# endernewton/tf-faster-rcnn

Measured on AMD Instinct MI355X. Metric: images/sec (600×1000) ResNet-101 Faster R-CNN at 1/2/4/8 MI355X, higher is better.
Workload: dtype f32 (operands, accumulators, results; GEMMs with Cin, Cout % 128 == 0 form each f32 product from two-piece fp16 operands with an exact power-of-two scale per 128-k block on the fp16 matrix pipe -- 3 MFMAs / product, dropped terms <= 3 * 2^-22, measured error vs float64 below the f32-MFMA kernel's; o

## Files before the change

### include/frcnn_hip.h

```cpp
#ifndef FRCNN_HIP_H_
#define FRCNN_HIP_H_
#include <stddef.h>
#include <stdint.h>

#ifdef __cplusplus
extern "C" {
#endif

#define FRCNN_OK 0
#define FRCNN_E_ARG (-1)
#define FRCNN_E_WS (-2)
#define FRCNN_E_UNSUPPORTED (-3)
#define FRCNN_E_HIP(e) (-(1000 + (int)(e)))

#define FRCNN_NMS_RULE_CPU 0
#define FRCNN_NMS_RULE_GPU 1

#define FRCNN_ACT_NONE 0
#define FRCNN_ACT_RELU 1
#define FRCNN_ACT_RELU6 2

#define FRCNN_ABI_VERSION 6
int frcnn_abi_version(void);
const char* frcnn_build_info(void);
// ... 87 lines not shown
size_t frcnn_conv2d_workspace_bytes(int N, int OH, int OW, int Cout, int KH, int KW, int Cin, int fold_w);
int frcnn_conv2d_nhwc_ws(const float* x_d, int N, int H, int W, int Cin, const float* w_d, const float* bias_d,
                         const float* residual_d, int RH, int RW, int res_stride, float* y_d, int OH, int OW, int Cout, int KH,
                         int KW, int stride, int pad_top, int pad_left, int act, int fold_w, void* ws, size_t ws_bytes,
                         void* stream);

int frcnn_set_tuning(int key, int value);
unsigned int frcnn_crc32c(const void* data, size_t n, unsigned int crc);

long long frcnn_snappy_uncompress(const unsigned char* src, size_t n, unsigned char* dst, size_t cap);

int frcnn_prep_image_shape(int h, int w, int target_size, int max_size, double* im_scale, int* out_h, int* out_w);
int frcnn_prep_image(const void* src_d, int src_is_float, int h, int w, const double* pixel_means, double im_scale, float* out_d,
                     int OH, int OW, int out_c, void* stream);
int frcnn_prep_train_image(const void* src_d, int src_is_float, int h, int w, int flipped, const double* pixel_means, double im_scale,
                           float* out_d, int OH, int OW, int out_c, const unsigned short* boxes_d, const int* classes_d, int G,
                           float* gt_d, void* stream);

int frcnn_gemm_batched_nt(const float* x_d, const float* w_d, float* y_d, int G, int M, int N, int K, void* stream);
size_t frcnn_gemm_x3_pack_bytes(int G, int N, int K);
int frcnn_gemm_x3_pack(const float* w_d, int G, int N, int K, void* planes_d, void* stream);
int frcnn_gemm_x3(const float* x_d, const void* planes_d, const float* bias_d, const float* res_d, float* y_d, int G, int M, int N,
                  int K, int act, int cfg, int terms, void* stream);
size_t frcnn_h2_planes_bytes(long long rows, int K);
int frcnn_h2_pack_w(const float* w_d, int G, int N, int K, void* planes_d, float* w_inv_d, void* stream);
int frcnn_h2_split(const float* x_d, long long M, int K, void* planes_d, float* inv_d, void* stream);
int frcnn_gemm_h2(const void* x_planes_d, const float* x_inv_d, const void* w_planes_d, const float* w_inv_d, const float* bias_d,
                  const float* res_d, const void* res_planes_d, const float* res_inv_d, float* y_d, void* y_planes_d, float* y_inv_d,
                  int G, int M, int N, int K, int act, int cfg, void* stream);
size_t frcnn_gemm_h2_mean_workspace_bytes(int G, int M, int N);
int frcnn_gemm_h2_mean(const void* x_planes_d, const float* x_inv_d, const void* w_planes_d, const float* w_inv_d, const float* bias_d,
                       const float* res_d, const void* res_planes_d, const float* res_inv_d, int G, int M, int N, int K, int act, int rows,
                       float* mean_out_d, void* ws, size_t ws_bytes, int cfg, void* stream);
int frcnn_winograd_filter_transform(const float* w_hwio, int Cin, int Cout, const float* scale, int m, float* u_out);
int frcnn_winograd_filter_transform_device(const float* w_packed_d, int Cout, int Cin, int m, int transpose_flip, float* u_d,
                                           void* stream);
int frcnn_winograd_input_transform(const float* x_d, int N, int H, int W, int C, int m, float* v_d, void* stream);
int frcnn_winograd_output_transform(const float* m_d, int N, int H, int W, int C, int m, const float* bias_d, int act, float* y_d,
                                    void* stream);
int frcnn_winograd7_filter_transform(const float* w_hwio, int Cin, int Cout, const float* scale, float* u_out);
int frcnn_winograd7_filter_transform_device(const float* w_packed_d, int Cout, int Cin, int transpose_flip, float* u_d, void* stream);
int frcnn_winograd7_input_transform(const float* x_d, int R, int C, float* v_d, void* stream);
int frcnn_winograd7_output_transform(const float* m_d, int R, int C, const float* bias_d, int act, float* y_d, void* stream);
int frcnn_winograd_input_transform_h2(const float* x_d, int N, int H, int W, int C, int m, void* v_planes_d, float* v_inv_d, void* stream);
int frcnn_winograd_output_transform_h2(const float* m_d, int N, int H, int W, int C, int m, const float* bias_d, int act, float* y_d,
                                       void* y_planes_d, float* y_inv_d, void* stream);
// ... 114 lines not shown
```

### tf-faster-rcnn_amd/csrc/gemm_h2.hip

```cpp
#include "h2_common.h"
#include <mutex>
#include <type_traits>

typedef float f32x16 __attribute__((ext_vector_type(16)));
typedef _Float16 h8 __attribute__((ext_vector_type(8)));

#define LDS_AS __attribute__((address_space(3)))

struct GemmH2Params {
  const unsigned short* x; const float* x_inv; const unsigned short* w; const float* w_inv;
  const float* bias; const float* res; const unsigned short* resp; const float* resp_inv; float* y; unsigned short* yp; float* y_inv;
  int M, N, K, batch, act, nsteps, mtiles, ntiles;
  long long Mtot;
  int wshare;
  const float* mask;
  float* mean_part; int mean_rows;
};

__device__ __forceinline__ void h2_glds16(unsigned voff, const void* sbase, unsigned lds_base) {
  unsigned keep;
  asm volatile(
      "s_mov_b32 %0, m0\n\t"
      "s_mov_b32 m0, %3\n\t"
      "s_nop 0\n\t"
// ... 1088 lines not shown
                                    const float* res_d, const float* mask_d, float* y_d, void* y_planes_d, float* y_inv_d, int G, int M, int N, int K,
                                    int act, int cfg, void* stream) {
  if (!x_planes_d || !x_inv_d || !w_planes_d || !w_inv_d || !mask_d || (!y_d && !y_planes_d) || (y_planes_d && !y_inv_d) || G <= 0 || M <= 0 ||
      N <= 0 || K <= 0 || act < 0 || act > 2)
    return FRCNN_E_ARG;
  const long long Mtot = (long long)G * M;
  if (K % H2_KB || N % 128 || 4ll * Mtot * K >= (1ll << 32) || 4ll * N * K >= (1ll << 32) || (long long)M * N >= (1ll << 29)) return FRCNN_E_UNSUPPORTED;
  GemmH2Params p = h2_params(x_planes_d, x_inv_d, w_planes_d, w_inv_d, bias_d, res_d, nullptr, nullptr, y_d, y_planes_d, y_inv_d, G, M, N, K, act);
  p.mask = mask_d;
  return run_h2(p, cfg, (hipStream_t)stream);
}

static int run_h2(GemmH2Params& p, int cfg, hipStream_t st) {
  const int G = p.batch, M = p.M, N = p.N, K = p.K;
  if (cfg < 0) {
    const long long mt256 = (M + 255) / 256;
#ifndef FRCNN_H2_PP_MIN_K
#define FRCNN_H2_PP_MIN_K 1024
#endif
    const int pp_min_k = ((cfg == -4 || cfg == -5 || cfg == -6) && !p.mean_part) ? 512 : FRCNN_H2_PP_MIN_K;
    const int pp_cfg = (cfg == -3 || cfg == -4 || (cfg == -6 && K < FRCNN_H2_PP_MIN_K)) ? 34 : 21;
    const bool pp = K >= pp_min_k && mt256 * 256 * 100 <= (long long)M * 104 && mt256 * (N / 128) * G >= 256;
    const bool tiny = (long long)((M + 127) / 128) * (N / 128) * G < 150;
    const bool de = cfg != -2 && cfg != -7 && !p.mean_part && !p.mask && ((p.resp && p.yp && !p.y) || cfg == -8);
    cfg = pp ? pp_cfg : tiny ? (cfg == -2 ? 12 : (de && cfg == -8) ? 41 : 33) : (cfg == -2 ? 9 : de ? 40 : 31);
  }
  if (p.mean_part && (cfg == 40 || cfg == 41)) cfg = cfg == 40 ? 31 : 33;
  return p.mask ? h2_dispatch<H2_MASKED>(p, cfg, st) : h2_dispatch<0>(p, cfg, st);
}

__global__ __launch_bounds__(256) void k_h2_mean_finish(const float* __restrict__ part, int G, int M, int N4, int rows, float4* __restrict__ out) {
  const long long t = (long long)blockIdx.x * blockDim.x + threadIdx.x;
  const int per = M / rows;
  if (t >= (long long)G * per * N4) return;
  const int n4 = (int)(t % N4);
  const long long gr = t / N4;
  const int g = (int)(gr / per), r = (int)(gr % per);
  const int nblk = (M + 31) >> 5;
  const int row0 = r * rows, row1 = row0 + rows - 1;
  float4 s = make_float4(0.f, 0.f, 0.f, 0.f);
  for (int b = row0 >> 5; b <= (row1 >> 5); ++b) {
    const int which = ((b << 5) / rows == r) ? 0 : 1;
    const float4 v = *(const float4*)(part + (((size_t)g * nblk + b) * 2 + which) * (size_t)N4 * 4 + (size_t)n4 * 4);
    s.x += v.x; s.y += v.y; s.z += v.z; s.w += v.w;
  }
  const float inv = 1.0f / (float)rows;
  out[t] = make_float4(s.x * inv, s.y * inv, s.z * inv, s.w * inv);
// ... 28 lines not shown
```

### tf-faster-rcnn_amd/csrc/gemm_x3.hip

```cpp
#include "common.h"
#include "mfma_f32.h"
#include <mutex>

typedef __attribute__((ext_vector_type(8))) __bf16 bf16x8;

struct GemmX3Params {
  const float* x; const unsigned short* wp; const float* bias; const float* res; float* y;
  int M, N, K, nsteps, mtiles, ntiles, batch, act;
  long long gx, gwp, gy;
};

__device__ __forceinline__ void x3_split8(const float4 a, const float4 b, bf16x8& h, bf16x8& m, bf16x8& l) {
  const float v[8] = {a.x, a.y, a.z, a.w, b.x, b.y, b.z, b.w};
#pragma unroll
  for (int q = 0; q < 8; ++q) {
    const __bf16 hq = (__bf16)v[q];
    const float r = v[q] - (float)hq;
    const __bf16 mq = (__bf16)r;
    const float s = r - (float)mq;
    h[q] = hq; m[q] = mq; l[q] = (__bf16)s;
  }
}

template <int BM, int BN, int WM, int WN, int TERMS = 6>
__global__ __launch_bounds__((BM / WM) * (BN / WN) * 64) __attribute__((amdgpu_waves_per_eu(2))) void k_gemm_x3(const GemmX3Params p) {
  constexpr int NW = (BM / WM) * (BN / WN);
  constexpr int TM = WM / 32, TN = WN / 32;
  constexpr int LA = BM / 8 / NW;
  constexpr int LB = 3 * BN / 16 / NW;
  constexpr int G = LA + LB;
  constexpr int A_BYTES = BM * 128, P_BYTES = BN * 64, STAGE = A_BYTES + 3 * P_BYTES;
  static_assert((BM / 8) % NW == 0 && (3 * BN / 16) % NW == 0, "tile/wave mismatch");
  extern __shared__ __attribute__((aligned(16))) char smem[];

  const int tid = threadIdx.x, lane = tid & 63;
  const int wave = __builtin_amdgcn_readfirstlane(tid >> 6);
  const int per = p.mtiles * p.ntiles, T = per * p.batch;
  const int xcd = blockIdx.x & 7, wx = blockIdx.x >> 3, W8 = gridDim.x >> 3;
  const int tq = T / 8, tr = T % 8, tn = tq + (xcd < tr ? 1 : 0);
  const int t_end = (xcd < tr ? xcd * (tq + 1) : tr * (tq + 1) + (xcd - tr) * tq) + tn;
  int tile = __builtin_amdgcn_readfirstlane(t_end - tn + wx);
  if (tile >= t_end) return;

  const int wm0 = (wave / (BN / WN)) * WM, wn0 = (wave % (BN / WN)) * WN;
  int a_lane[LA], b_lane[LB];
#pragma unroll
  for (int t = 0; t < LB; ++t) {
    const int u = wave * LB + t;
    const int plane = u / (BN / 16), row = (u % (BN / 16)) * 16 + (lane >> 2), pos = lane & 3;
    b_lane[t] = ((plane * p.N + row) * p.K) * 2 + ((pos ^ ((row >> 2) & 3)) * 16);
  }
  const float* ia = p.x; const char* ib = (const char*)p.wp;
  int i_bm0 = 0, i_bn0 = 0, i_g = 0;
  auto set_tile = [&](int tl) {
    const int g = tl / per, rem = tl - g * per;
    const int mt = rem / p.ntiles, nt = rem - mt * p.ntiles;
    i_bm0 = mt * BM; i_bn0 = nt * BN; i_g = g;
    ia = p.x + (size_t)g * p.gx + (size_t)i_bm0 * p.K;
    ib = (const char*)(p.wp + (size_t)g * p.gwp + (size_t)i_bn0 * p.K);
#pragma unroll
    for (int t = 0; t < LA; ++t) {
      const int row = (wave * LA + t) * 8 + (lane >> 3);
      a_lane[t] = (min(row, p.M - 1 - i_bm0) * p.K + ((lane & 7) ^ ((row >> 1) & 7)) * 4) * 4;
    }
  };
  const unsigned lds0 = (unsigned)(size_t)(LDS_AS char*)smem;
  auto issue_one = [&](int buf, int t) {
    const unsigned sb = lds0 + (unsigned)(buf * STAGE);
    if (t < LA) glds16((const char*)ia + a_lane[t], __builtin_amdgcn_readfirstlane(sb + (wave * LA + t) * 1024));
    else glds16(ib + b_lane[t - LA], __builtin_amdgcn_readfirstlane(sb + A_BYTES + (wave * LB + (t - LA)) * 1024));
  };
  auto advance_k = [&]() { ia += 32; ib += 64; };
  auto issue_slab = [&](int buf) {
#pragma unroll
    for (int t = 0; t < G; ++t) issue_one(buf, t);
    advance_k();
  };

  f32x16 acc[TM][TN], acs[TM][TN];
  auto zero_acc = [&]() {
#pragma unroll
    for (int i = 0; i < TM; ++i)
#pragma unroll
      for (int j = 0; j < TN; ++j)
#pragma unroll
        for (int r = 0; r < 16; ++r) { acc[i][j][r] = 0.f; acs[i][j][r] = 0.f; }
  };
  zero_acc();
  const int frow = lane & 31, khalf = lane >> 5;
  const int a_sw = (frow >> 1) & 7, b_sw = (frow >> 2) & 3;
  const int a_row = (wm0 + frow) * 128, b_row = A_BYTES + (wn0 + frow) * 64;

  int c_bm0, c_bn0, c_g;
  const int lane_off = (4 * khalf * p.N + frow) * 4;
  auto sub_base = [&](int i, int j) { return (long long)(c_bm0 + wm0 + i * 32) * p.N + (long long)(c_bn0 + wn0 + j * 32); };
// ... 32 lines not shown
          acs[i][j] = __builtin_amdgcn_mfma_f32_32x32x16_bf16(al[i], bh[j], acs[i][j], 0, 0, 0);
          acc[i][j] = __builtin_amdgcn_mfma_f32_32x32x16_bf16(ah[i], bh[j], acc[i][j], 0, 0, 0);
          acs[i][j] = __builtin_amdgcn_mfma_f32_32x32x16_bf16(ah[i], bl[j], acs[i][j], 0, 0, 0);
          acs[i][j] = __builtin_amdgcn_mfma_f32_32x32x16_bf16(am[i], bm[j], acs[i][j], 0, 0, 0);
          acs[i][j] = __builtin_amdgcn_mfma_f32_32x32x16_bf16(am[i], bh[j], acs[i][j], 0, 0, 0);
          acs[i][j] = __builtin_amdgcn_mfma_f32_32x32x16_bf16(ah[i], bm[j], acs[i][j], 0, 0, 0);
          if (TERMS == 9) {
            acs[i][j] = __builtin_amdgcn_mfma_f32_32x32x16_bf16(al[i], bl[j], acs[i][j], 0, 0, 0);
            acs[i][j] = __builtin_amdgcn_mfma_f32_32x32x16_bf16(al[i], bm[j], acs[i][j], 0, 0, 0);
            acs[i][j] = __builtin_amdgcn_mfma_f32_32x32x16_bf16(am[i], bl[j], acs[i][j], 0, 0, 0);
          }
        }
    }
    advance_k();
  };

  const float act_lo = p.act == FRCNN_ACT_NONE ? -__builtin_inff() : 0.f;
  const float act_hi = p.act == FRCNN_ACT_RELU6 ? 6.f : __builtin_inff();
  auto finish = [&](auto res_c) {
    constexpr bool RES = decltype(res_c)::value;
    float* const py = p.y + (size_t)c_g * p.gy;
    int lo = lane_off;
    asm volatile("" : "+v"(lo));
#pragma unroll
    for (int i = 0; i < TM; ++i)
#pragma unroll
      for (int j = 0; j < TN; ++j) {
        const float bv = p.bias ? p.bias[c_bn0 + wn0 + j * 32 + frow] : 0.f;
        const long long sbase = sub_base(i, j);
        float v[16];
        if (RES) {
          const auto rr = rsrc_of(p.res + (size_t)c_g * p.gy, sbase);
#pragma unroll
          for (int r = 0; r < 16; ++r) v[r] = __builtin_bit_cast(float, __builtin_amdgcn_raw_buffer_load_b32(rr, lo + row_soff(r), 0, 0));
        }
#pragma unroll
        for (int r = 0; r < 16; ++r) {
          float t = (acc[i][j][r] + acs[i][j][r]) + bv;
          if (RES) t += v[r];
          v[r] = act_clamp(t, act_lo, act_hi);
        }
        const auto ry = rsrc_of(py, sbase);
#pragma unroll
        for (int r = 0; r < 16; ++r) __builtin_amdgcn_raw_buffer_store_b32(__builtin_bit_cast(unsigned, v[r]), ry, lo + row_soff(r), 0, 0);
      }
  };

  set_tile(tile);
  c_bm0 = i_bm0; c_bn0 = i_bn0; c_g = i_g;
  issue_slab(0);
  int cur = 0, step = 0;
  for (;;) {
    wait_vmcnt<0>();
    __builtin_amdgcn_s_barrier();
// ... 20 lines not shown
  const long long g = i / nk, e = i - g * nk;
  const float x = w[i];
  const __bf16 h = (__bf16)x;
  const float r = x - (float)h;
  const __bf16 m = (__bf16)r;
  const __bf16 l = (__bf16)(r - (float)m);
  unsigned short* o = out + (size_t)g * 3 * nk + e;
  o[0] = __builtin_bit_cast(unsigned short, h); o[nk] = __builtin_bit_cast(unsigned short, m); o[2 * nk] = __builtin_bit_cast(unsigned short, l);
}

extern "C" size_t frcnn_gemm_x3_pack_bytes(int G, int N, int K) {
  if (G <= 0 || N <= 0 || K <= 0) return 0;
  return (size_t)G * 3 * (size_t)N * (size_t)K * sizeof(unsigned short);
}

extern "C" int frcnn_gemm_x3_pack(const float* w_d, int G, int N, int K, void* planes_d, void* stream) {
  if (!w_d || !planes_d || G <= 0 || N <= 0 || K <= 0) return FRCNN_E_ARG;
  const long long nk = (long long)N * K, tot = nk * G;
  hipLaunchKernelGGL(k_x3_pack, dim3((unsigned)((tot + 255) / 256)), dim3(256), 0, (hipStream_t)stream, w_d, nk, G, (unsigned short*)planes_d);
  LAUNCH_CHECK();
  return FRCNN_OK;
}

template <int BM, int BN, int WM, int WN, int TERMS = 6>
static int launch_x3(const GemmX3Params& q, hipStream_t st) {
  constexpr int NT = (BM / WM) * (BN / WN) * 64;
  constexpr size_t lds = 2 * (size_t)(BM * 128 + 3 * BN * 64);
  auto kern = k_gemm_x3<BM, BN, WM, WN, TERMS>;
  static KernelOnce once;
  int slots = 0;
  HIP_TRY(kernel_once(once, (const void*)kern, NT, lds, &slots));
  if (slots < 8 || q.N % BN) return FRCNN_E_UNSUPPORTED;
  GemmX3Params p = q;
  p.mtiles = cdiv(p.M, BM); p.ntiles = p.N / BN; p.nsteps = p.K / 32;
  const long long T = (long long)p.mtiles * p.ntiles * p.batch;
  if (T >= (1ll << 30)) return FRCNN_E_UNSUPPORTED;
  const int grid = (int)min((long long)(slots / 8) * 8, ((T + 7) / 8) * 8);
  hipLaunchKernelGGL(kern, dim3(grid), dim3(NT), lds, st, p);
  LAUNCH_CHECK();
  return FRCNN_OK;
}

extern "C" int frcnn_gemm_x3(const float* x_d, const void* planes_d, const float* bias_d, const float* res_d, float* y_d, int G, int M,
                             int N, int K, int act, int cfg, int terms, void* stream) {
  if (!x_d || !planes_d || !y_d || G <= 0 || M <= 0 || N <= 0 || K <= 0 || act < 0 || act > 2 || (terms != 6 && terms != 9)) return FRCNN_E_ARG;
  if (K % 32 || N % 64 || (long long)M * N >= (1ll << 31) || (long long)N * K >= (1ll << 28) || K >= (1 << 22))
    return FRCNN_E_UNSUPPORTED;
  GemmX3Params p;
  p.x = x_d; p.wp = (const unsigned short*)planes_d; p.bias = bias_d; p.res = res_d; p.y = y_d;
  p.M = M; p.N = N; p.K = K; p.batch = G; p.act = act;
  p.gx = (long long)M * K; p.gwp = 3ll * N * K; p.gy = (long long)M * N;
  p.nsteps = p.mtiles = p.ntiles = 0;
  hipStream_t st = (hipStream_t)stream;
  if (cfg >= 0 && cfg < 10 && (N % 128) && cfg != 6) cfg = -1;
  if (cfg < 0)
    cfg = (N % 128) ? 6 : ((long long)cdiv(M, 128) * (N / 128) * G >= 256) ? 0 : 1;
  if (terms == 9) {
    switch (cfg) {
      case 0: return launch_x3<128, 128, 64, 64, 9>(p, st);
      case 1: return launch_x3<128, 128, 32, 64, 9>(p, st);
      case 6: return launch_x3<128, 64, 64, 32, 9>(p, st);
      default: return FRCNN_E_ARG;
    }
  }
  switch (cfg) {
    case 0: return launch_x3<128, 128, 64, 64>(p, st);
    case 1: return launch_x3<128, 128, 32, 64>(p, st);
    case 2: return launch_x3<64, 128, 32, 64>(p, st);
    case 3: return launch_x3<128, 128, 32, 128>(p, st);
    case 4: return launch_x3<256, 128, 64, 64>(p, st);
    case 5: return launch_x3<128, 256, 64, 64>(p, st);
    case 6: return launch_x3<128, 64, 64, 32>(p, st);
    default: return FRCNN_E_ARG;
  }
}
```

### tf-faster-rcnn_amd/frcnn_hip/__init__.py

```python
import ctypes
import os
from ctypes import c_double, c_float, c_int, c_longlong, c_size_t, c_ulonglong, c_void_p

_PKG = os.path.dirname(os.path.abspath(__file__))
LIB_PATH = os.path.join(_PKG, "libfrcnn_hip.so")
_lib = None

ABI_VERSION = 6
ACT_NONE, ACT_RELU, ACT_RELU6 = 0, 1, 2
NMS_RULE_CPU, NMS_RULE_GPU = 0, 1

_P = c_void_p
SIGNATURES = {
    "frcnn_abi_version": (c_int, []),
    "frcnn_build_info": (ctypes.c_char_p, []),
    "_nms": (None, [_P, _P, _P, c_int, c_int, c_float, c_int]),
    "frcnn_nms_workspace_bytes": (c_size_t, [c_int]),
    "frcnn_nms": (c_int, [_P, c_int, c_double, c_int, _P, _P, _P, c_size_t, _P]),
    "frcnn_nms_sorted": (c_int, [_P, c_int, c_int, c_double, c_int, _P, _P, _P, c_size_t, _P]),
    "frcnn_nms_rule": (c_int, [_P, c_int, c_double, c_int, c_int, _P, _P, _P, c_size_t, _P]),
    "frcnn_nms_sorted_rule": (c_int, [_P, c_int, c_int, c_double, c_int, c_int, _P, _P, _P, c_size_t, _P]),
    "frcnn_generate_anchors": (c_int, [c_int, _P, c_int, _P, c_int, _P]),
    "frcnn_generate_anchors_pre": (c_int, [c_int, c_int, c_int, _P, c_int, _P, _P]),
    "frcnn_proposal_workspace_bytes": (c_size_t, [c_int, c_int, c_int, c_int]),
# ... 75 lines not shown
    "frcnn_proposal_target_layer_dn": (c_int, [_P, _P, c_int, _P, _P, c_int, c_int, c_int, c_double, c_double, c_double, c_double, _P, _P,
                                               c_longlong, _P, _P, _P, _P, _P, _P, _P, _P, _P]),
    "frcnn_loss_workspace_bytes": (c_size_t, [c_longlong]),
    "frcnn_softmax_ce_loss": (c_int, [_P, _P, c_int, c_int, c_int, c_int, c_int, _P, _P, _P, c_size_t, _P]),
    "frcnn_smooth_l1_loss": (c_int, [_P, _P, _P, _P, c_longlong, c_float, c_float, _P, _P, _P, c_size_t, _P]),
    "frcnn_transpose_pad": (c_int, [_P, c_int, c_int, _P, c_int, _P]),
    "frcnn_im2col_t": (c_int, [_P, c_int, c_int, c_int, c_int, c_int, c_int, c_int, c_int, c_int, c_int, c_int, _P, c_int, _P]),
    "frcnn_flip_transpose_filter": (c_int, [_P, c_int, c_int, c_int, c_int, _P, _P]),
    "frcnn_conv2d_dgrad_strided": (c_int, [_P, c_int, c_int, c_int, c_int, _P, c_int, c_int, c_int, c_int, c_int, c_int, _P, c_int,
                                           c_int, c_int, _P]),
    "frcnn_conv2d_wgrad_supported": (c_int, [c_int, c_int]),
    "frcnn_conv2d_wgrad_workspace_bytes": (c_size_t, [c_int, c_int, c_int, c_int, c_int, c_int, c_int]),
    "frcnn_conv2d_wgrad": (c_int, [_P, _P, c_int, c_int, c_int, c_int, c_int, c_int, c_int, c_int, c_int, c_int, c_int, c_int, _P, _P,
                                   c_size_t, _P]),
    "frcnn_conv2d_wgrad_set_plan": (None, [c_int, c_int]),
    "frcnn_conv2d_wgrad_h2_workspace_bytes": (c_size_t, [c_int, c_int, c_int, c_int, c_int, c_int, c_int]),
    "frcnn_conv2d_wgrad_h2": (c_int, [_P, _P, c_int, c_int, c_int, c_int, c_int, c_int, c_int, c_int, c_int, c_int, c_int, c_int, _P, _P,
                                      c_size_t, _P]),
    "frcnn_conv2d_wgrad_h2_set_plan": (None, [c_int, c_int]),
    "frcnn_relu_bwd": (c_int, [_P, _P, c_longlong, _P]),
    "frcnn_gemm_x3_pack_bytes": (c_size_t, [c_int, c_int, c_int]),
    "frcnn_gemm_x3_pack": (c_int, [_P, c_int, c_int, c_int, _P, _P]),
    "frcnn_gemm_x3": (c_int, [_P, _P, _P, _P, _P, c_int, c_int, c_int, c_int, c_int, c_int, c_int, _P]),
    "frcnn_h2_planes_bytes": (c_size_t, [c_longlong, c_int]),
    "frcnn_h2_pack_w": (c_int, [_P, c_int, c_int, c_int, _P, _P, _P]),
    "frcnn_h2_split": (c_int, [_P, c_longlong, c_int, _P, _P, _P]),
    "frcnn_gemm_h2": (c_int, [_P, _P, _P, _P, _P, _P, _P, _P, _P, _P, _P, c_int, c_int, c_int, c_int, c_int, c_int, _P]),
    "frcnn_gemm_h2_mean_workspace_bytes": (c_size_t, [c_int, c_int, c_int]),
    "frcnn_gemm_h2_mean": (c_int, [_P, _P, _P, _P, _P, _P, _P, _P, c_int, c_int, c_int, c_int, c_int, c_int, _P, _P, c_size_t, c_int, _P]),
    "frcnn_relu6_bwd": (c_int, [_P, _P, c_longlong, _P]),
    "frcnn_maxpool_bwd": (c_int, [_P, c_int, c_int, c_int, c_int, c_int, c_int, _P, _P, c_int, c_int, _P, _P]),
    "frcnn_dropout": (c_int, [_P, c_longlong, c_ulonglong, c_float, _P, _P]),
    "frcnn_dwconv3x3_dgrad": (c_int, [_P, c_int, c_int, c_int, c_int, _P, _P, c_int, c_int, c_int, c_int, c_int, c_int, _P]),
    "frcnn_dwconv3x3_wgrad_workspace_bytes": (c_size_t, [c_int, c_int, c_int, c_int]),
    "frcnn_dwconv3x3_wgrad": (c_int, [_P, _P, c_int, c_int, c_int, c_int, c_int, c_int, c_int, c_int, c_int, _P, _P, _P, c_size_t, _P]),
    "frcnn_dwconv3x3_refold": (c_int, [_P, _P, c_int, _P, _P]),
    "frcnn_add_strided": (c_int, [_P, c_int, c_int, c_int, c_int, _P, c_int, c_int, c_int, c_int, _P]),
    "frcnn_spatial_mean_bwd": (c_int, [_P, c_int, c_int, c_int, _P, _P]),
    "frcnn_colsum": (c_int, [_P, c_int, c_int, _P, _P]),
    "frcnn_crop_and_resize_bwd": (c_int, [_P, c_int, c_int, c_int, _P, c_int, c_float, c_int, _P, _P]),
    "frcnn_crop_and_resize_bwd_plan": (c_int, [_P, c_int, c_int, c_int, _P, c_int, c_float, c_int, _P, c_size_t, _P]),
    "frcnn_sgd_momentum": (c_int, [_P, _P, _P, _P, _P, c_longlong, c_int, c_float, c_float, c_float, c_float, _P]),
    "frcnn_sgd_desc_bytes": (c_size_t, []),
    "frcnn_sgd_momentum_multi": (c_int, [_P, c_int, c_float, c_float, c_float, _P]),
    "frcnn_sgd_momentum_range": (c_int, [_P, c_int, c_int, c_float, c_float, c_float, _P]),
    "frcnn_sumsq": (c_int, [_P, c_longlong, c_double, _P, c_int, _P, c_size_t, _P]),
# ... 47 lines not shown
```

### tf-faster-rcnn_amd/frcnn_hip/ops.py

```python
import ctypes

import numpy as np
import torch

import frcnn_hip as _binding
from . import ACT_NONE, NMS_RULE_CPU, call, lib

_ws_cache = {}
ws_scope = "default"

_scope_stack = [(None, None, None)]


def active_store(owner, default=None):
    o, _, store = _scope_stack[-1]
    return store if store is not None and (owner is None or o is owner) else default


def scope_depth():
    return len(_scope_stack) - 1


class unscoped(object):

# ... 795 lines not shown
def relu_bwd(grad, y):
    _chk(grad), _chk(y)
    call("frcnn_relu_bwd", _ptr(grad), _ptr(y), grad.numel(), _stream())
    return grad


def gemm_x3_pack(w, planes=None):
    _chk(w)
    G, N, K = (w.shape[0], w.shape[1], w.shape[2]) if w.dim() == 3 else (1, w.shape[0], w[0].numel())
    if planes is None:
        planes = torch.empty(lib().frcnn_gemm_x3_pack_bytes(G, N, K), dtype=torch.uint8, device=w.device)
    call("frcnn_gemm_x3_pack", _ptr(w), G, N, K, _ptr(planes), _stream())
    return planes


def gemm_x3(x, planes, G, M, N, K, bias=None, residual=None, act=ACT_NONE, out=None, cfg=-1, terms=6):
    _chk(x)
    out = _empty((G, M, N) if G > 1 else (M, N), dtype=torch.float32, device=x.device) if out is None else out
    call("frcnn_gemm_x3", _ptr(x), _ptr(planes), _ptr(bias), _ptr(residual), _ptr(out), int(G), int(M), int(N), int(K), int(act),
         int(cfg), int(terms), _stream())
    return out


class H2(object):
    __slots__ = ("planes", "inv", "rows", "K")

    def __init__(self, planes, inv, rows, K):
        self.planes, self.inv, self.rows, self.K = planes, inv, int(rows), int(K)

    @staticmethod
    def empty(rows, K, device):
        assert K % 128 == 0
        return H2(torch.empty(lib().frcnn_h2_planes_bytes(int(rows), int(K)), dtype=torch.uint8, device=device),
                  torch.empty((K // 128, rows), dtype=torch.float32, device=device), rows, K)

    def to_float(self):
        hl = self.planes.view(torch.float16).view(2, self.rows, self.K).float()
        inv = self.inv.t().repeat_interleave(128, dim=1)
        return (hl[0] + hl[1]) * inv


def h2_split(x, out=None):
    _chk(x)
    K = x.shape[-1]
    rows = x.numel() // K
    out = H2.empty(rows, K, x.device) if out is None else out
# ... 218 lines not shown
```

### tf-faster-rcnn_amd/lib/model/config.py

```python
import ast
import os
import os.path as osp

import numpy as np


class AttrDict(dict):

    def __init__(self, d=None, **kw):
        super().__init__()
        for k, v in dict(d or {}, **kw).items():
            self[k] = v

    def __setitem__(self, k, v):
        if isinstance(v, dict) and not isinstance(v, AttrDict):
            v = AttrDict(v)
        super().__setitem__(k, v)

    def __getattr__(self, k):
        try:
            return self[k]
        except KeyError:
            raise AttributeError(k)

# ... 9 lines not shown
    BBOX_INSIDE_WEIGHTS=(1.0, 1.0, 1.0, 1.0), BBOX_NORMALIZE_TARGETS_PRECOMPUTED=True,
    BBOX_NORMALIZE_MEANS=(0.0, 0.0, 0.0, 0.0), BBOX_NORMALIZE_STDS=(0.1, 0.1, 0.2, 0.2), PROPOSAL_METHOD='gt',
    HAS_RPN=True, RPN_POSITIVE_OVERLAP=0.7, RPN_NEGATIVE_OVERLAP=0.3, RPN_CLOBBER_POSITIVES=False,
    RPN_FG_FRACTION=0.5, RPN_BATCHSIZE=256, RPN_NMS_THRESH=0.7, RPN_PRE_NMS_TOP_N=12000,
    RPN_POST_NMS_TOP_N=2000, RPN_BBOX_INSIDE_WEIGHTS=(1.0, 1.0, 1.0, 1.0), RPN_POSITIVE_WEIGHT=-1.0,
    USE_ALL_GT=True)

_TEST = dict(
    SCALES=(600,), MAX_SIZE=1000, NMS=0.3, SVM=False, BBOX_REG=True, HAS_RPN=False, PROPOSAL_METHOD='gt',
    RPN_NMS_THRESH=0.7, RPN_PRE_NMS_TOP_N=6000, RPN_POST_NMS_TOP_N=300, MODE='nms', RPN_TOP_N=5000)

__C = AttrDict(
    TRAIN=_TRAIN, TEST=_TEST,
    RESNET=dict(MAX_POOL=False, FIXED_BLOCKS=1),
    MOBILENET=dict(REGU_DEPTH=False, FIXED_LAYERS=5, WEIGHT_DECAY=0.00004, DEPTH_MULTIPLIER=1.),
    PIXEL_MEANS=np.array([[[102.9801, 115.9465, 122.7717]]]), RNG_SEED=3,
    ROOT_DIR=osp.abspath(osp.join(osp.dirname(__file__), '..', '..')),
    MATLAB='matlab', EXP_DIR='default', USE_GPU_NMS=True, USE_E2E_TF=False, POOLING_MODE='crop', POOLING_SIZE=7,
    ANCHOR_SCALES=[8, 16, 32], ANCHOR_RATIOS=[0.5, 1, 2], RPN_CHANNELS=512,
    HIP=dict(WINOGRAD=True, WINOGRAD_MIN_CIN=64, WINOGRAD_M=4, WINOGRAD_F2_SCOPES=("block1", "block2"), WINOGRAD_DIRECT_SCOPES=(),
             WINOGRAD_TRAIN=True, WINOGRAD_DGRAD=True,
             WINOGRAD_7X7=True, FUSE_TAIL_MEAN=True, MFMA_X3=True,
             MFMA_H2=True, H2_LAZY_SPLIT=True, H2_MIN_TILES=150, H2_TRAIN_MIN_TILES=320, H2_TRUNK_PLANES=True, H2_TILE_CFG=-1,
             X3_TILE_CFG=-1, H2_TRAIN=True, WGRAD_STREAM=2, WGRAD_TN=True, WGRAD_H2=True, PREP_STREAM=True, TRAIN_REPLAY=True, TRAIN_PICK_STREAMS=6,
             GRAPH_CACHE_SHAPES=4, TRAIN_CACHE_SHAPES=16))
__C.DATA_DIR = osp.abspath(osp.join(__C.ROOT_DIR, 'data'))
cfg = __C


def get_output_dir(imdb, weights_filename):
    outdir = osp.abspath(osp.join(__C.ROOT_DIR, 'output', __C.EXP_DIR, imdb.name))
    outdir = osp.join(outdir, 'default' if weights_filename is None else weights_filename)
    os.makedirs(outdir, exist_ok=True)
    return outdir


def get_output_tb_dir(imdb, weights_filename):
    outdir = osp.abspath(osp.join(__C.ROOT_DIR, 'tensorboard', __C.EXP_DIR, imdb.name))
    outdir = osp.join(outdir, 'default' if weights_filename is None else weights_filename)
    os.makedirs(outdir, exist_ok=True)
    return outdir


_NULLABLE_KEYS = ("H2_TRAIN_MIN_TILES",)


def _merge_a_into_b(a, b):
# ... 56 lines not shown
```

### tf-faster-rcnn_amd/lib/nets/network.py

```python
import collections

import numpy as np
import torch

from frcnn_hip import ACT_NONE, ACT_RELU, NMS_RULE_CPU, NMS_RULE_GPU, ops
from frcnn_hip.runtime import VarSpec
from model.config import cfg


class Network(object):
    def __init__(self):
        self._predictions = {}
        self._losses = {}
        self._anchor_targets = {}
        self._proposal_targets = {}
        self._layers = {}
        self._act_summaries = []
        self._variables_to_fix = {}
        self._feat_stride = [16, ]
        self._scope = "network"
        self._sess = None
        self._image = None
        self._im_info = None
        self._var_specs = collections.OrderedDict()
# ... 71 lines not shown
                      lambda: ops.conv3x3_winograd(x, u, b, act, out=out, v_buf=v, m_buf=mm, out_planes=yp),
                      nbytes=4 * (v.numel() + u.numel() + mm.numel()))
            self._wrote(out, yp, True) if yp is not None else self._wrote(out)
        elif plain and self._h2_eligible(M, Cout, Cin, 1, scope) and self._h2_input(x) is not None:
            xp, wp = self._h2_input(x), sess.h2_planes(w)
            yp = sess.h2_buf(self._tag + "/" + scope, M, Cout) if emit_h2 else None
            y = out if (want_f32 or yp is None or self._mode == "TRAIN") else None
            res = residual
            if residual is not None and residual.data_ptr() in self._f32_missing:
                res = self._h2_of[residual.data_ptr()]
            tcfg = int(cfg.HIP.H2_TILE_CFG)
            sess.mark("conv:h2:" + scope, flops, lambda: ops.gemm_h2(xp, wp, 1, M, Cout, Cin, b, res, act, out=y, out_planes=yp,
                                                                      want_f32=False, cfg=tcfg),
                      nbytes=4 * M * Cin + 4 * w.numel() + (4 * out.numel() if y is not None else 0)
                      + (4 * out.numel() if yp is not None else 0) + (4 * out.numel() if residual is not None else 0))
            self._wrote(out, yp, y is not None)
        elif plain and self._x3_eligible(M, Cout, Cin, 1):
            self._need_f32(x), self._need_f32(residual)
            planes = sess.x3_planes(w)
            xc = int(cfg.HIP.X3_TILE_CFG)
            sess.mark("conv:x3:" + scope, flops, lambda: ops.gemm_x3(x, planes, 1, M, Cout, Cin, b, residual, act, out=out, cfg=xc),
                      nbytes=4 * (x.numel() + out.numel() + (out.numel() if residual is not None else 0)) + 6 * w.numel())
            self._wrote(out)
        else:
            self._need_f32(x), self._need_f32(residual)
            sess.mark("conv:" + scope, flops,
                      lambda: ops.conv2d(x, w, b, k, k, stride, pad, act, residual, res_stride, fold_w, out=out),
                      nbytes=4 * (x.numel() + w.numel() + out.numel() + (out.numel() if residual is not None else 0)))
            self._wrote(out)
        if self._mode == "TRAIN":
            self._tape.append(dict(kind="conv", scope=scope, x=x, y=out, k=k, stride=stride, pad=tuple(pad), act=act,
                                   residual=residual, res_stride=res_stride))
            if self.trainable_scope(scope) or x.data_ptr() in self._requires_grad:
                self._requires_grad.add(out.data_ptr())
            if residual is not None and residual.data_ptr() in self._requires_grad:
                self._requires_grad.add(out.data_ptr())
        return out

    H2_MIN_CHANNEL_RATIO = 2.0 ** -18

    def _h2_eligible(self, M, N, K, G, scope=None):
        rows = G * M
        if scope is not None and self._mode == "TEST" and self._sess.h2_channel_spread(scope) < self.H2_MIN_CHANNEL_RATIO:
            return False
        return (bool(cfg.HIP.MFMA_H2) and (self._mode == "TEST" or bool(cfg.HIP.H2_TRAIN)) and K % 128 == 0 and N % 128 == 0
                and ((self._plan_rows(M) + 127) // 128) * (N // 128) * G >= self._h2_min_tiles()
# ... 14 lines not shown
            self._need_f32(x)
            K = x.shape[-1]
            xp = self._sess.h2_buf(self._tag + "/split@%x" % x.data_ptr(), x.numel() // K, K)
            self._sess.mark("op:h2_split", 0, lambda: ops.h2_split(x, out=xp), nbytes=8 * x.numel())
            self._h2_of[x.data_ptr()] = xp
        return xp

    def _wrote(self, t, planes=None, f32=True):
        k = t.data_ptr()
        if planes is None:
            self._h2_of.pop(k, None)
        else:
            self._h2_of[k] = planes
        (self._f32_missing.discard if f32 else self._f32_missing.add)(k)
        return t

    def _need_f32(self, x):
        if x is not None and x.data_ptr() in self._f32_missing:
            raise RuntimeError("graph construction error: a float32 consumer reads a tensor that was emitted as operand planes only")

    def _x3_eligible(self, M, N, K, G):
        return (bool(cfg.HIP.MFMA_X3) and self._mode == "TEST" and N % 64 == 0 and K % 32 == 0
                and ((self._plan_rows(M) + 127) // 128) * ((N + 127) // 128) * G >= 150 and M * N < (1 << 31) and N * K < (1 << 28))

    @staticmethod
    def _winograd_scheme(scope, H, W):
        if any(tok in scope for tok in cfg.HIP.WINOGRAD_F2_SCOPES):
            return 2
        m = int(cfg.HIP.WINOGRAD_M)
        return 7 if (m == 4 and H == 7 and W == 7 and cfg.HIP.WINOGRAD_7X7) else m

    def _conv_winograd(self, x, scope, act, bn_eps, emit_h2=False, want_f32=True):
        sess = self._sess
        self._need_f32(x)
        N, H, W, Cin = x.shape
        m = self._winograd_scheme(scope, H, W)
        u, b = sess.winograd_params(scope, bn_eps=bn_eps, m=m)
        G, Cout = u.shape[0], u.shape[1]
        T = ops.winograd_tiles(N, H, W, m)
        mm = sess.buf(self._tag + "/wino_m", (G, T, Cout))
        out = sess.buf(self._tag + "/" + scope, (N, H, W, Cout))
        flops = 2 * G * T * Cout * Cin
        if self._h2_eligible(T, Cout, Cin, G, scope):
            vp, wp = sess.h2_buf(self._tag + "/wino_v", G * T, Cin), sess.h2_planes(u)
            sess.mark("op:wino_in", 0, lambda: ops.winograd_input_transform_h2(x, vp, m), nbytes=4 * (x.numel() + G * T * Cin))
            tcfg = int(cfg.HIP.H2_TILE_CFG)
# ... 353 lines not shown
        self._var(self._scope + "/bbox_pred/biases", (4 * num_classes,), "zeros")
        names = ["rois", "rpn_cls_score", "rpn_cls_prob", "rpn_bbox_pred", "cls_score", "cls_prob", "bbox_pred"]
        return {k: k for k in names}

    def _stage_image(self, sess, image, im_info=None):
        if isinstance(image, np.ndarray):
            image = torch.from_numpy(np.ascontiguousarray(image, dtype=np.float32))
        B, H, W, C = image.shape
        if im_info is None:
            buf = sess.buf(self._tag + "/image", (B, H, W, 4), zero=True)
        else:
            with self.shape_scope(sess, (B, H, W, 4), im_info):
                buf = sess.buf(self._tag + "/image", (B, H, W, 4), zero=True)
        buf[..., :C].copy_(image, non_blocking=True)
        return buf

    def graph_key(self, image_shape, im_info):
        c = cfg[self._mode]
        return (self._tag, self._scope, self._num_classes, self._anchor_scales, self._anchor_ratios, bool(cfg.RESNET.MAX_POOL),
                bool(cfg.USE_GPU_NMS), tuple(int(v) for v in image_shape), (float(im_info[0]), float(im_info[1])), self._mode, cfg.TEST.MODE, self._fuse_tail_entry,
                c.RPN_PRE_NMS_TOP_N, c.RPN_POST_NMS_TOP_N, c.RPN_NMS_THRESH, cfg.TEST.RPN_TOP_N, cfg.POOLING_SIZE,
                bool(cfg.HIP.WINOGRAD), int(cfg.HIP.WINOGRAD_MIN_CIN), int(cfg.HIP.WINOGRAD_M), tuple(cfg.HIP.WINOGRAD_F2_SCOPES),
                tuple(cfg.HIP.WINOGRAD_DIRECT_SCOPES), bool(cfg.HIP.WINOGRAD_7X7), bool(cfg.HIP.FUSE_TAIL_MEAN), bool(cfg.HIP.MFMA_X3), bool(cfg.USE_E2E_TF),
                bool(cfg.HIP.MFMA_H2), bool(cfg.HIP.H2_LAZY_SPLIT), int(cfg.HIP.H2_MIN_TILES), bool(cfg.HIP.H2_TRUNK_PLANES), int(cfg.HIP.H2_TILE_CFG), int(cfg.HIP.X3_TILE_CFG), bool(cfg.HIP.H2_TRAIN))

    def shape_scope(self, sess, image_shape, im_info):
        return sess.shape_scope(self.graph_key(image_shape, im_info), group=("graphs", self._tag), cap=int(cfg.HIP.GRAPH_CACHE_SHAPES))

    def forward_device(self, sess, image_d, im_info, use_graph=True):
        self._sess = sess
        self._image = image_d
        self._im_info = (float(im_info[0]), float(im_info[1]), float(im_info[2]))
        sess.prepared.wait_planes()
        ops.ws_scope = self._tag
        key = self.graph_key(image_d.shape, self._im_info)
        cur = torch.cuda.current_stream(sess.device)
        with self.shape_scope(sess, image_d.shape, self._im_info):
            if not use_graph or sess.profile is not None:
                sess.flops_last_forward = 0
                self._build_network(self._mode == "TRAIN")
                return self._predictions
            if key not in sess.graphs:
                with torch.cuda.stream(sess.stream):
                    sess.stream.wait_stream(cur)
                    sess.flops_last_forward = 0
                    self._build_network(False)
                    sess.stream.synchronize()
# ... 249 lines not shown
```

Baseline: 546.8.

## Route stem, stride-2 3x3 and strided-residual 1x1 convs through implicit-GEMM x3 kernel

Adds an implicit-GEMM convolution mode to the x3 (three-plane bf16 MFMA) GEMM kernel. It gathers input patches directly into LDS with zero-fill for padding, supports a folded-width stem, and adds a strided-residual epilogue mode for 1x1 convs whose residual is read at stride 2. The network now routes stem, stride-2 3x3 and res2-class convs to this path, which were previously handled by the generic conv kernel. The h2 dual-emit config is also restricted to K<512. The gather adds per-lane address arithmetic, and the per-element residual offsets raise register pressure.

```diff
diff --git a/include/frcnn_hip.h b/include/frcnn_hip.h
--- a/include/frcnn_hip.h
+++ b/include/frcnn_hip.h
@@ -133,6 +133,9 @@
 int frcnn_gemm_x3_pack(const float* w_d, int G, int N, int K, void* planes_d, void* stream);
 int frcnn_gemm_x3(const float* x_d, const void* planes_d, const float* bias_d, const float* res_d, float* y_d, int G, int M, int N,
                   int K, int act, int cfg, int terms, void* stream);
+int frcnn_conv2d_x3(const float* x_d, int N, int H, int W, int Cin, const void* planes_d, const float* bias_d, const float* residual_d,
+                    int RH, int RW, int res_stride, float* y_d, int OH, int OW, int Cout, int KH, int KW, int stride, int pad_top,
+                    int pad_left, int act, int fold_w, int cfg, void* stream);
 size_t frcnn_h2_planes_bytes(long long rows, int K);
 int frcnn_h2_pack_w(const float* w_d, int G, int N, int K, void* planes_d, float* w_inv_d, void* stream);
 int frcnn_h2_split(const float* x_d, long long M, int K, void* planes_d, float* inv_d, void* stream);
diff --git a/tf-faster-rcnn_amd/csrc/gemm_h2.hip b/tf-faster-rcnn_amd/csrc/gemm_h2.hip
--- a/tf-faster-rcnn_amd/csrc/gemm_h2.hip
+++ b/tf-faster-rcnn_amd/csrc/gemm_h2.hip
@@ -1134,7 +1134,7 @@
     const int pp_cfg = (cfg == -3 || cfg == -4 || (cfg == -6 && K < FRCNN_H2_PP_MIN_K)) ? 34 : 21;
     const bool pp = K >= pp_min_k && mt256 * 256 * 100 <= (long long)M * 104 && mt256 * (N / 128) * G >= 256;
     const bool tiny = (long long)((M + 127) / 128) * (N / 128) * G < 150;
-    const bool de = cfg != -2 && cfg != -7 && !p.mean_part && !p.mask && ((p.resp && p.yp && !p.y) || cfg == -8);
+    const bool de = cfg != -2 && cfg != -7 && !p.mean_part && !p.mask && ((p.resp && p.yp && !p.y && K < 512) || cfg == -8);
     cfg = pp ? pp_cfg : tiny ? (cfg == -2 ? 12 : (de && cfg == -8) ? 41 : 33) : (cfg == -2 ? 9 : de ? 40 : 31);
   }
   if (p.mean_part && (cfg == 40 || cfg == 41)) cfg = cfg == 40 ? 31 : 33;
diff --git a/tf-faster-rcnn_amd/csrc/gemm_x3.hip b/tf-faster-rcnn_amd/csrc/gemm_x3.hip
--- a/tf-faster-rcnn_amd/csrc/gemm_x3.hip
+++ b/tf-faster-rcnn_amd/csrc/gemm_x3.hip
@@ -8,7 +8,12 @@
   const float* x; const unsigned short* wp; const float* bias; const float* res; float* y;
   int M, N, K, nsteps, mtiles, ntiles, batch, act;
   long long gx, gwp, gy;
+  int H, W, OH, OW, pixb, stride, pad_top, pad_left, KW, CB, fold;
+  int RH, RW, rs, res_bytes;
 };
+
+enum { X3_GATHER = 1, X3_RSTRIDE = 2 };
+__device__ float4 g_x3_zero[4];
 
 __device__ __forceinline__ void x3_split8(const float4 a, const float4 b, bf16x8& h, bf16x8& m, bf16x8& l) {
   const float v[8] = {a.x, a.y, a.z, a.w, b.x, b.y, b.z, b.w};
@@ -22,7 +27,7 @@
   }
 }
 
-template <int BM, int BN, int WM, int WN, int TERMS = 6>
+template <int BM, int BN, int WM, int WN, int TERMS = 6, int MODE = 0>
 __global__ __launch_bounds__((BM / WM) * (BN / WN) * 64) __attribute__((amdgpu_waves_per_eu(2))) void k_gemm_x3(const GemmX3Params p) {
   constexpr int NW = (BM / WM) * (BN / WN);
   constexpr int TM = WM / 32, TN = WN / 32;
@@ -43,7 +48,11 @@
   if (tile >= t_end) return;
 
   const int wm0 = (wave / (BN / WN)) * WM, wn0 = (wave % (BN / WN)) * WN;
+  constexpr bool GATHER = (MODE & X3_GATHER) != 0, RSTRIDE = (MODE & X3_RSTRIDE) != 0;
   int a_lane[LA], b_lane[LB];
+  int a_iy[GATHER ? LA : 1], a_ix[GATHER ? LA : 1];
+  int g_kh = 0, g_kw = 0, g_cb = 0;
+  const int ohow = (GATHER || RSTRIDE) ? p.OH * p.OW : 1;
 #pragma unroll
   for (int t = 0; t < LB; ++t) {
     const int u = wave * LB + t;
@@ -56,8 +65,21 @@
     const int g = tl / per, rem = tl - g * per;
     const int mt = rem / p.ntiles, nt = rem - mt * p.ntiles;
     i_bm0 = mt * BM; i_bn0 = nt * BN; i_g = g;
+    ib = (const char*)(p.wp + (size_t)g * p.gwp + (size_t)i_bn0 * p.K);
+    if constexpr (GATHER) {
+      ia = p.x; g_kh = g_kw = g_cb = 0;
+#pragma unroll
+      for (int t = 0; t < LA; ++t) {
+        const int row = (wave * LA + t) * 8 + (lane >> 3), m = i_bm0 + row, chunk = (lane & 7) ^ ((row >> 1) & 7);
+        const int b = m / ohow, rem = m - b * ohow, oy = rem / p.OW, ox = rem - oy * p.OW;
+        const int iy = oy * p.stride - p.pad_top, ix = ox * p.stride - p.pad_left + (p.fold ? chunk : 0);
+        a_iy[t] = (m < p.M && (!p.fold || chunk < p.fold)) ? iy : -(1 << 28);
+        a_ix[t] = ix;
+        a_lane[t] = ((b * p.H + iy) * p.W + ix) * p.pixb + (p.fold ? 0 : chunk * 16);
+      }
+      return;
+    }
     ia = p.x + (size_t)g * p.gx + (size_t)i_bm0 * p.K;
-    ib = (const char*)(p.wp + (size_t)g * p.gwp + (size_t)i_bn0 * p.K);
 #pragma unroll
     for (int t = 0; t < LA; ++t) {
       const int row = (wave * LA + t) * 8 + (lane >> 3);
@@ -67,10 +89,23 @@
   const unsigned lds0 = (unsigned)(size_t)(LDS_AS char*)smem;
   auto issue_one = [&](int buf, int t) {
     const unsigned sb = lds0 + (unsigned)(buf * STAGE);
+    if constexpr (GATHER) {
+      if (t < LA) {
+        const bool ok = (unsigned)(a_iy[t] + g_kh) < (unsigned)p.H && (unsigned)(a_ix[t] + g_kw) < (unsigned)p.W;
+        glds16(ok ? (const char*)ia + a_lane[t] : (const char*)g_x3_zero, __builtin_amdgcn_readfirstlane(sb + (wave * LA + t) * 1024));
+        return;
+      }
+    }
     if (t < LA) glds16((const char*)ia + a_lane[t], __builtin_amdgcn_readfirstlane(sb + (wave * LA + t) * 1024));
     else glds16(ib + b_lane[t - LA], __builtin_amdgcn_readfirstlane(sb + A_BYTES + (wave * LB + (t - LA)) * 1024));
   };
-  auto advance_k = [&]() { ia += 32; ib += 64; };
+  auto advance_k = [&]() {
+    ib += 64;
+    if (GATHER) {
+      if (++g_cb == p.CB) { g_cb = 0; if (++g_kw == p.KW) { g_kw = 0; ++g_kh; } }
+      ia = (const float*)((const char*)p.x + ((long long)(g_kh * p.W + g_kw) * p.pixb + g_cb * 128));
+    } else ia += 32;
+  };
   auto issue_slab = [&](int buf) {
 #pragma unroll
     for (int t = 0; t < G; ++t) issue_one(buf, t);
@@ -149,6 +184,24 @@
     float* const py = p.y + (size_t)c_g * p.gy;
     int lo = lane_off;
     asm volatile("" : "+v"(lo));
+    int roff[RSTRIDE ? TM : 1][16];
+    const auto res_rs = __builtin_amdgcn_make_buffer_rsrc((void*)p.res, 0, RSTRIDE ? p.res_bytes : 0, 0x00020000);
+    if constexpr (RES && RSTRIDE) {
+      const int stepx = p.rs * p.N * 4, wrapx = (p.RW - p.OW) * stepx, wrapy = (p.RH - p.OH * p.rs) * p.RW * p.N * 4;
+#pragma unroll
+      for (int i = 0; i < TM; ++i) {
+        const int m0 = c_bm0 + wm0 + i * 32 + 4 * khalf;
+        const int b = m0 / ohow, rem = m0 - b * ohow;
+        int oy = rem / p.OW, ox = rem - oy * p.OW;
+        int off = ((b * p.RH + oy * p.rs) * p.RW + ox * p.rs) * p.N * 4;
+#pragma unroll
+        for (int d = 0; d < 28; ++d) {
+          if (!(d & 4)) roff[i][(d & 3) + 4 * (d >> 3)] = off;
+          off += stepx;
+          if (++ox == p.OW) { ox = 0; off += wrapx; if (++oy == p.OH) { oy = 0; off += wrapy; } }
+        }
+      }
+    }
 #pragma unroll
     for (int i = 0; i < TM; ++i)
 #pragma unroll
@@ -156,7 +209,11 @@
         const float bv = p.bias ? p.bias[c_bn0 + wn0 + j * 32 + frow] : 0.f;
         const long long sbase = sub_base(i, j);
         float v[16];
-        if (RES) {
+        if constexpr (RES && RSTRIDE) {
+          const int cb4 = (c_bn0 + wn0 + j * 32 + frow) * 4;
+#pragma unroll
+          for (int r = 0; r < 16; ++r) v[r] = __builtin_bit_cast(float, __builtin_amdgcn_raw_buffer_load_b32(res_rs, roff[i][r] + cb4, 0, 0));
+        } else if (RES) {
           const auto rr = rsrc_of(p.res + (size_t)c_g * p.gy, sbase);
 #pragma unroll
           for (int r = 0; r < 16; ++r) v[r] = __builtin_bit_cast(float, __builtin_amdgcn_raw_buffer_load_b32(rr, lo + row_soff(r), 0, 0));
@@ -223,11 +280,11 @@
   return FRCNN_OK;
 }
 
-template <int BM, int BN, int WM, int WN, int TERMS = 6>
+template <int BM, int BN, int WM, int WN, int TERMS = 6, int MODE = 0>
 static int launch_x3(const GemmX3Params& q, hipStream_t st) {
   constexpr int NT = (BM / WM) * (BN / WN) * 64;
   constexpr size_t lds = 2 * (size_t)(BM * 128 + 3 * BN * 64);
-  auto kern = k_gemm_x3<BM, BN, WM, WN, TERMS>;
+  auto kern = k_gemm_x3<BM, BN, WM, WN, TERMS, MODE>;
   static KernelOnce once;
   int slots = 0;
   HIP_TRY(kernel_once(once, (const void*)kern, NT, lds, &slots));
@@ -242,20 +299,21 @@
   return FRCNN_OK;
 }
 
+static int x3_cfg_by_shape(int G, int M, int N) { return (N % 128) ? 6 : ((long long)cdiv(M, 128) * (N / 128) * G >= 256) ? 0 : 1; }
+
 extern "C" int frcnn_gemm_x3(const float* x_d, const void* planes_d, const float* bias_d, const float* res_d, float* y_d, int G, int M,
                              int N, int K, int act, int cfg, int terms, void* stream) {
   if (!x_d || !planes_d || !y_d || G <= 0 || M <= 0 || N <= 0 || K <= 0 || act < 0 || act > 2 || (terms != 6 && terms != 9)) return FRCNN_E_ARG;
   if (K % 32 || N % 64 || (long long)M * N >= (1ll << 31) || (long long)N * K >= (1ll << 28) || K >= (1 << 22))
     return FRCNN_E_UNSUPPORTED;
-  GemmX3Params p;
+  GemmX3Params p = {};
   p.x = x_d; p.wp = (const unsigned short*)planes_d; p.bias = bias_d; p.res = res_d; p.y = y_d;
   p.M = M; p.N = N; p.K = K; p.batch = G; p.act = act;
   p.gx = (long long)M * K; p.gwp = 3ll * N * K; p.gy = (long long)M * N;
   p.nsteps = p.mtiles = p.ntiles = 0;
   hipStream_t st = (hipStream_t)stream;
   if (cfg >= 0 && cfg < 10 && (N % 128) && cfg != 6) cfg = -1;
-  if (cfg < 0)
-    cfg = (N % 128) ? 6 : ((long long)cdiv(M, 128) * (N / 128) * G >= 256) ? 0 : 1;
+  if (cfg < 0) cfg = x3_cfg_by_shape(G, M, N);
   if (terms == 9) {
     switch (cfg) {
       case 0: return launch_x3<128, 128, 64, 64, 9>(p, st);
@@ -275,3 +333,49 @@
     default: return FRCNN_E_ARG;
   }
 }
+
+template <int MODE>
+static int x3_dispatch_geom(const GemmX3Params& p, int cfg, hipStream_t st) {
+  switch (cfg) {
+    case 0: return launch_x3<128, 128, 64, 64, 6, MODE>(p, st);
+    case 1: return launch_x3<128, 128, 32, 64, 6, MODE>(p, st);
+    case 6: return launch_x3<128, 64, 64, 32, 6, MODE>(p, st);
+    default: return FRCNN_E_ARG;
+  }
+}
+
+extern "C" int frcnn_conv2d_x3(const float* x_d, int N, int H, int W, int Cin, const void* planes_d, const float* bias_d,
+                               const float* residual_d, int RH, int RW, int res_stride, float* y_d, int OH, int OW, int Cout, int KH, int KW,
+                               int stride, int pad_top, int pad_left, int act, int fold_w, int cfg, void* stream) {
+  if (!x_d || !planes_d || !y_d) return FRCNN_E_ARG;
+  if (N <= 0 || H <= 0 || W <= 0 || Cin <= 0 || OH <= 0 || OW <= 0 || Cout <= 0 || KH <= 0 || KW <= 0 || stride <= 0 || pad_top < 0 || pad_left < 0)
+    return FRCNN_E_ARG;
+  if (act < 0 || act > 2) return FRCNN_E_ARG;
+  if (residual_d && (res_stride < 1 || RH < (OH - 1) * res_stride + 1 || RW < (OW - 1) * res_stride + 1)) return FRCNN_E_ARG;
+  if (fold_w) {
+    if (Cin != 4 || KW > 8) return FRCNN_E_UNSUPPORTED;
+  } else if (Cin % 32) {
+    return FRCNN_E_UNSUPPORTED;
+  }
+  const long long M = (long long)N * OH * OW, K = fold_w ? (long long)KH * 32 : (long long)KH * KW * Cin;
+  if (Cout % 64 || (long long)N * H * W * Cin * 4 >= (1ll << 31) || M * Cout >= (1ll << 31) || (long long)Cout * K >= (1ll << 28) || K >= (1 << 22) ||
+      M + 256 >= (1ll << 31))
+    return FRCNN_E_UNSUPPORTED;
+  const bool strided_res = residual_d && res_stride != 1;
+  const bool plain = !fold_w && KH == 1 && KW == 1 && stride == 1 && pad_top == 0 && pad_left == 0 && OH == H && OW == W;
+  if (plain && !strided_res)
+    return frcnn_gemm_x3(x_d, planes_d, bias_d, residual_d, y_d, 1, (int)M, Cout, (int)K, act, cfg, 6, stream);
+  if (!plain && strided_res) return FRCNN_E_UNSUPPORTED;
+  if (strided_res && (long long)(N + 2) * RH * RW * Cout * 4 >= (1ll << 31)) return FRCNN_E_UNSUPPORTED;
+  GemmX3Params p;
+  p.x = x_d; p.wp = (const unsigned short*)planes_d; p.bias = bias_d; p.res = residual_d; p.y = y_d;
+  p.M = (int)M; p.N = Cout; p.K = (int)K; p.batch = 1; p.act = act;
+  p.gx = 0; p.gwp = 3ll * Cout * K; p.gy = M * Cout;
+  p.nsteps = p.mtiles = p.ntiles = 0;
+  p.H = H; p.W = W; p.OH = OH; p.OW = OW; p.pixb = Cin * 4; p.stride = stride; p.pad_top = pad_top; p.pad_left = pad_left;
+  p.KW = fold_w ? 1 : KW; p.CB = fold_w ? 1 : Cin / 32; p.fold = fold_w ? KW : 0;
+  p.RH = RH; p.RW = RW; p.rs = res_stride; p.res_bytes = strided_res ? (int)((long long)N * RH * RW * Cout * 4) : 0;
+  if ((cfg != 0 && cfg != 1 && cfg != 6) || (cfg != 6 && Cout % 128)) cfg = -1;
+  if (cfg < 0) cfg = x3_cfg_by_shape(1, (int)M, Cout);
+  return plain ? x3_dispatch_geom<X3_RSTRIDE>(p, cfg, (hipStream_t)stream) : x3_dispatch_geom<X3_GATHER>(p, cfg, (hipStream_t)stream);
+}
diff --git a/tf-faster-rcnn_amd/frcnn_hip/__init__.py b/tf-faster-rcnn_amd/frcnn_hip/__init__.py
--- a/tf-faster-rcnn_amd/frcnn_hip/__init__.py
+++ b/tf-faster-rcnn_amd/frcnn_hip/__init__.py
@@ -121,6 +121,8 @@
     "frcnn_gemm_x3_pack_bytes": (c_size_t, [c_int, c_int, c_int]),
     "frcnn_gemm_x3_pack": (c_int, [_P, c_int, c_int, c_int, _P, _P]),
     "frcnn_gemm_x3": (c_int, [_P, _P, _P, _P, _P, c_int, c_int, c_int, c_int, c_int, c_int, c_int, _P]),
+    "frcnn_conv2d_x3": (c_int, [_P, c_int, c_int, c_int, c_int, _P, _P, _P, c_int, c_int, c_int, _P, c_int, c_int, c_int, c_int, c_int,
+                                c_int, c_int, c_int, c_int, c_int, c_int, _P]),
     "frcnn_h2_planes_bytes": (c_size_t, [c_longlong, c_int]),
     "frcnn_h2_pack_w": (c_int, [_P, c_int, c_int, c_int, _P, _P, _P]),
     "frcnn_h2_split": (c_int, [_P, c_longlong, c_int, _P, _P, _P]),
diff --git a/tf-faster-rcnn_amd/frcnn_hip/ops.py b/tf-faster-rcnn_amd/frcnn_hip/ops.py
--- a/tf-faster-rcnn_amd/frcnn_hip/ops.py
+++ b/tf-faster-rcnn_amd/frcnn_hip/ops.py
@@ -841,6 +841,22 @@
     return out
 
 
+def conv2d_x3(x, planes, bias, Cout, KH, KW, stride=1, pad=(0, 0, 0, 0), act=ACT_NONE, residual=None, res_stride=1, fold_w=False,
+              out=None, cfg=-1):
+    _chk(x)
+    N, H, W, Cin = x.shape
+    OH = conv_out_size(H, KH, stride, pad[0], pad[1])
+    OW = conv_out_size(W, KW, stride, pad[2], pad[3])
+    out = _empty((N, OH, OW, Cout), dtype=torch.float32, device=x.device) if out is None else out
+    RH = RW = 0
+    if residual is not None:
+        _chk(residual)
+        RH, RW = residual.shape[1], residual.shape[2]
+    call("frcnn_conv2d_x3", _ptr(x), N, H, W, Cin, _ptr(planes), _ptr(bias), _ptr(residual), RH, RW, int(res_stride), _ptr(out), OH, OW,
+         int(Cout), KH, KW, int(stride), int(pad[0]), int(pad[2]), int(act), 1 if fold_w else 0, int(cfg), _stream())
+    return out
+
+
 class H2(object):
     __slots__ = ("planes", "inv", "rows", "K")
 
diff --git a/tf-faster-rcnn_amd/lib/model/config.py b/tf-faster-rcnn_amd/lib/model/config.py
--- a/tf-faster-rcnn_amd/lib/model/config.py
+++ b/tf-faster-rcnn_amd/lib/model/config.py
@@ -55,7 +55,7 @@
              WINOGRAD_TRAIN=True, WINOGRAD_DGRAD=True,
              WINOGRAD_7X7=True, FUSE_TAIL_MEAN=True, MFMA_X3=True,
              MFMA_H2=True, H2_LAZY_SPLIT=True, H2_MIN_TILES=150, H2_TRAIN_MIN_TILES=320, H2_TRUNK_PLANES=True, H2_TILE_CFG=-1,
-             X3_TILE_CFG=-1, H2_TRAIN=True, WGRAD_STREAM=2, WGRAD_TN=True, WGRAD_H2=True, PREP_STREAM=True, TRAIN_REPLAY=True, TRAIN_PICK_STREAMS=6,
+             X3_TILE_CFG=-1, X3_CONV=("stem", "s2", "res2"), H2_TRAIN=True, WGRAD_STREAM=2, WGRAD_TN=True, WGRAD_H2=True, PREP_STREAM=True, TRAIN_REPLAY=True, TRAIN_PICK_STREAMS=6,
              GRAPH_CACHE_SHAPES=4, TRAIN_CACHE_SHAPES=16))
 __C.DATA_DIR = osp.abspath(osp.join(__C.ROOT_DIR, 'data'))
 cfg = __C
diff --git a/tf-faster-rcnn_amd/lib/nets/network.py b/tf-faster-rcnn_amd/lib/nets/network.py
--- a/tf-faster-rcnn_amd/lib/nets/network.py
+++ b/tf-faster-rcnn_amd/lib/nets/network.py
@@ -117,6 +117,14 @@
             sess.mark("conv:x3:" + scope, flops, lambda: ops.gemm_x3(x, planes, 1, M, Cout, Cin, b, residual, act, out=out, cfg=xc),
                       nbytes=4 * (x.numel() + out.numel() + (out.numel() if residual is not None else 0)) + 6 * w.numel())
             self._wrote(out)
+        elif self._x3_conv_class(k, stride, pad, fold_w, Cin, Cout, M, residual is not None, res_stride) is not None:
+            self._need_f32(x), self._need_f32(residual)
+            planes = sess.x3_planes(w)
+            xc = int(cfg.HIP.X3_TILE_CFG)
+            sess.mark("conv:x3:" + scope, flops,
+                      lambda: ops.conv2d_x3(x, planes, b, Cout, k, k, stride, pad, act, residual, res_stride, fold_w, out=out, cfg=xc),
+                      nbytes=4 * (x.numel() + out.numel() + (out.numel() if residual is not None else 0)) + 6 * w.numel())
+            self._wrote(out)
         else:
             self._need_f32(x), self._need_f32(residual)
             sess.mark("conv:" + scope, flops,
@@ -177,6 +185,17 @@
     def _x3_eligible(self, M, N, K, G):
         return (bool(cfg.HIP.MFMA_X3) and self._mode == "TEST" and N % 64 == 0 and K % 32 == 0
                 and ((self._plan_rows(M) + 127) // 128) * ((N + 127) // 128) * G >= 150 and M * N < (1 << 31) and N * K < (1 << 28))
+
+    def _x3_conv_class(self, k, stride, pad, fold_w, Cin, Cout, M, has_residual, res_stride):
+        if fold_w:
+            cls, K = "stem", k * 32
+        elif k == 3 and stride == 2 and not has_residual and Cin % 32 == 0:
+            cls, K = "s2", 9 * Cin
+        elif k == 1 and stride == 1 and tuple(pad) == (0, 0, 0, 0) and has_residual and res_stride == 2 and Cin % 32 == 0:
+            cls, K = "res2", Cin
+        else:
+            return None
+        return cls if (cls in tuple(cfg.HIP.X3_CONV) and self._x3_eligible(M, Cout, K, 1)) else None
 
     @staticmethod
     def _winograd_scheme(scope, H, W):
@@ -576,7 +595,8 @@
                 c.RPN_PRE_NMS_TOP_N, c.RPN_POST_NMS_TOP_N, c.RPN_NMS_THRESH, cfg.TEST.RPN_TOP_N, cfg.POOLING_SIZE,
                 bool(cfg.HIP.WINOGRAD), int(cfg.HIP.WINOGRAD_MIN_CIN), int(cfg.HIP.WINOGRAD_M), tuple(cfg.HIP.WINOGRAD_F2_SCOPES),
                 tuple(cfg.HIP.WINOGRAD_DIRECT_SCOPES), bool(cfg.HIP.WINOGRAD_7X7), bool(cfg.HIP.FUSE_TAIL_MEAN), bool(cfg.HIP.MFMA_X3), bool(cfg.USE_E2E_TF),
-                bool(cfg.HIP.MFMA_H2), bool(cfg.HIP.H2_LAZY_SPLIT), int(cfg.HIP.H2_MIN_TILES), bool(cfg.HIP.H2_TRUNK_PLANES), int(cfg.HIP.H2_TILE_CFG), int(cfg.HIP.X3_TILE_CFG), bool(cfg.HIP.H2_TRAIN))
+                bool(cfg.HIP.MFMA_H2), bool(cfg.HIP.H2_LAZY_SPLIT), int(cfg.HIP.H2_MIN_TILES), bool(cfg.HIP.H2_TRUNK_PLANES), int(cfg.HIP.H2_TILE_CFG), int(cfg.HIP.X3_TILE_CFG), bool(cfg.HIP.H2_TRAIN),
+                tuple(cfg.HIP.X3_CONV))
 
     def shape_scope(self, sess, image_shape, im_info):
         return sess.shape_scope(self.graph_key(image_shape, im_info), group=("graphs", self._tag), cap=int(cfg.HIP.GRAPH_CACHE_SHAPES))
```

Result: no change. 552.1, median of 6 (+1.0%).
